# yukiteruono/pbsim3

Hardware: AMD Instinct MI355X
Metric: simulated bases/sec (higher is better)
Workload: dtype u8

## Files before the change

pbsim3_amd/csrc/deflate.hip:

```cpp
#include <hip/hip_runtime.h>
#include <stdint.h>
#include <stdlib.h>

#include "kernels.h"

namespace pbsim {

namespace {

constexpr int kChunk = DF_CHUNK;
constexpr int kThreads = 256;
constexpr int kSeg = kChunk / kThreads;
constexpr int kSegDw = kSeg / 4;
constexpr int kInDw = kChunk / 4 + kChunk / 128;
constexpr int kOutBytes = 33024;
constexpr int kOutDw = kOutBytes / 4;
constexpr int kSyms = 288;
constexpr uint32_t kPoly = 0xEDB88320u;
constexpr int kHeadBits = 18 * 8;
constexpr int kPrefixBits = 3 + 5 + 5 + 4 + 19 * 3;

constexpr int kClLenTab[19] = {3, 5, 4, 4, 4, 5, 5, 5, 5, 5, 5, 5, 4, 5, 5, 5, 5, 3, 3};
constexpr int kClOrderTab[19] = {16, 17, 18, 0, 8, 7, 9, 6, 10, 5, 11, 4, 12, 3, 13, 2, 14, 1, 15};
constexpr uint64_t pack_cl_len() {
  uint64_t v = 0;
  for (int s = 0; s < 19; ++s) v |= (uint64_t)kClLenTab[s] << (3 * s);
  return v;
}
constexpr uint64_t kClLenPacked = pack_cl_len();
__device__ __forceinline__ uint32_t cl_len(uint32_t s) { return (uint32_t)(kClLenPacked >> (3 * s)) & 7u; }
constexpr unsigned __int128 pack_prefix() {
  unsigned __int128 v = 1u | (2u << 1) | ((unsigned __int128)15 << 13);
  for (int i = 0; i < 19; ++i) v |= (unsigned __int128)kClLenTab[kClOrderTab[i]] << (17 + 3 * i);
  return v;
}
constexpr uint64_t kPrefixLo = (uint64_t)pack_prefix();
constexpr uint32_t kPrefixHi = (uint32_t)(pack_prefix() >> 64);

__device__ __forceinline__ uint32_t rev_bits(uint32_t code, uint32_t len) { return __brev(code) >> (32 - len); }

__device__ __forceinline__ uint32_t cl_code(uint32_t s) {
  uint32_t c, l = cl_len(s);
  if (l == 3) c = s == 0 ? 0 : s - 16;
  else if (l == 4) c = s == 12 ? 9 : 4 + s;
  else c = s == 1 ? 20 : s <= 11 ? 16 + s : 15 + s;
  return rev_bits(c, l);
}

__device__ __forceinline__ uint32_t gf2_mul(uint32_t a, uint32_t b) {
  uint32_t p = 0;
#pragma unroll
  for (int i = 0; i < 32; ++i) {
    p ^= b & (0u - ((a >> (31 - i)) & 1u));
    b = (b >> 1) ^ (kPoly & (0u - (b & 1u)));
  }
  return p;
}

struct BitWriter {
  uint32_t *out;
  uint32_t word, nb;
  uint64_t acc;
  __device__ __forceinline__ void init(uint32_t *o, uint32_t bitpos) {
    out = o;
    word = bitpos >> 5;
    nb = bitpos & 31;
    acc = 0;
  }
  __device__ __forceinline__ void put(uint32_t v, uint32_t k) {
    acc |= (uint64_t)v << nb;
    nb += k;
    if (nb >= 32) {
      atomicOr(&out[word++], (uint32_t)acc);
      acc >>= 32;
      nb -= 32;
    }
  }
  __device__ __forceinline__ void put64(uint64_t v, uint32_t k) {
    if (k > 32) {
      put((uint32_t)v, 32);
      put((uint32_t)(v >> 32), k - 32);
    } else {
      put((uint32_t)v, k);
    }
  }
  __device__ __forceinline__ void flush() {
    if (nb) atomicOr(&out[word], (uint32_t)acc);
  }
};

__device__ __forceinline__ void length_symbol(uint32_t L, uint32_t *sym, uint32_t *eb, uint32_t *ev) {
  const uint32_t v = L - 3;
  if (v < 8) {
    *sym = 257 + v;
    *eb = 0;
    *ev = 0;
  } else if (L == 258) {
    *sym = 285;
    *eb = 0;
    *ev = 0;
  } else {
    const uint32_t e = (31 - __clz(v)) - 2;
    *sym = 261 + 4 * e + ((v >> e) & 3);
    *eb = e;
    *ev = v & ((1u << e) - 1);
  }
}

__device__ __forceinline__ uint32_t block_scan_excl(uint32_t v, uint32_t *s_wave, uint32_t *total) {
  const int lane = threadIdx.x & 63, wave = threadIdx.x >> 6;
  uint32_t inc = v;
#pragma unroll
  for (int d = 1; d < 64; d <<= 1) {
    const uint32_t o = __shfl_up(inc, d, 64);
    if (lane >= d) inc += o;
  }
  __syncthreads();
  if (lane == 63) s_wave[wave] = inc;
  __syncthreads();
  uint32_t base = 0, tot = 0;
#pragma unroll
  for (int w = 0; w < kThreads / 64; ++w) {
    const uint32_t x = s_wave[w];
    if (w < wave) base += x;
    tot += x;
  }
  *total = tot;
  return base + inc - v;
}

struct Mask128 {
  uint64_t lo, hi;
};
__device__ __forceinline__ Mask128 m_and(Mask128 a, Mask128 b) { return {a.lo & b.lo, a.hi & b.hi}; }
__device__ __forceinline__ Mask128 m_or(Mask128 a, Mask128 b) { return {a.lo | b.lo, a.hi | b.hi}; }
__device__ __forceinline__ Mask128 m_not(Mask128 a) { return {~a.lo, ~a.hi}; }
template <int K>
__device__ __forceinline__ Mask128 m_shl(Mask128 a) { return {a.lo << K, (a.hi << K) | (a.lo >> (64 - K))}; }
template <int K>
__device__ __forceinline__ Mask128 m_shr(Mask128 a) { return {(a.lo >> K) | (a.hi << (64 - K)), a.hi >> K}; }
__device__ __forceinline__ uint32_t m_nibble(Mask128 a, int j) {
  return (uint32_t)((j < 16 ? a.lo >> (4 * j) : a.hi >> (4 * j - 64)) & 15u);
}
__device__ __forceinline__ int m_first(Mask128 a) { return a.lo ? __builtin_ctzll(a.lo) : 64 + __builtin_ctzll(a.hi); }
__device__ __forceinline__ Mask128 m_clear(Mask128 a, int pos) {
  if (pos < 64) a.lo &= ~(1ull << pos);
  else a.hi &= ~(1ull << (pos - 64));
  return a;
}
__device__ __forceinline__ int m_run(Mask128 m, int pos) {
  uint64_t lo, hi;
  if (pos == 0) {
    lo = m.lo;
    hi = m.hi;
  } else if (pos < 64) {
    lo = (m.lo >> pos) | (m.hi << (64 - pos));
    hi = m.hi >> pos;
  } else {
    lo = m.hi >> (pos - 64);
    hi = 0;
  }
  if (~lo) return __builtin_ctzll(~lo);
  return ~hi ? 64 + __builtin_ctzll(~hi) : 128;
}

struct SegTokens {
  Mask128 lit;
  Mask128 start;
  Mask128 cover;
};

__device__ __forceinline__ SegTokens seg_tokens(const uint32_t (&seg)[kSegDw], int seg_n, uint32_t prev_dword,
                                                bool chunk_start) {
  uint64_t e[2] = {0, 0};
  uint32_t pw = prev_dword;
#pragma unroll
  for (int j = 0; j < kSegDw; ++j) {
    const uint32_t w = seg[j];
    const uint32_t d = w ^ ((w << 8) | (pw >> 24));
    const uint32_t z = ~(((d & 0x7F7F7F7Fu) + 0x7F7F7F7Fu) | d | 0x7F7F7F7Fu);
    const uint32_t nib = (((z >> 7) * 0x00204081u) >> 21) & 15u;
    e[j >> 4] |= (uint64_t)nib << (4 * (j & 15));
    pw = w;
  }
  Mask128 valid;
  valid.lo = seg_n >= 64 ? ~0ull : (1ull << seg_n) - 1;
  valid.hi = seg_n >= 128 ? ~0ull : seg_n > 64 ? (1ull << (seg_n - 64)) - 1 : 0ull;
  Mask128 eq = {e[0] & valid.lo, e[1] & valid.hi};
  if (chunk_start) eq.lo &= ~1ull;
  const Mask128 r3 = m_and(eq, m_and(m_shr<1>(eq), m_shr<2>(eq)));
  SegTokens t;
  t.cover = m_or(r3, m_or(m_shl<1>(r3), m_shl<2>(r3)));
  t.start = m_and(t.cover, m_not(m_shl<1>(t.cover)));
  t.lit = m_and(valid, m_not(t.cover));
  return t;
}

constexpr int kSampleChunks = DF_SAMPLE_CHUNKS;
constexpr int kHdrDw = DF_TABLE_HDR_DW;

struct DfTable {
  uint32_t code[kSyms];
  uint32_t hdr_end_bits;
  uint32_t pad[3];
  uint32_t hdr[kHdrDw];
};
static_assert(sizeof(DfTable) <= DF_TABLE_BYTES, "DF_TABLE_BYTES too small");

__device__ __forceinline__ void load_chunk(const uint8_t *__restrict__ text, int64_t n_bytes, int64_t chunk, uint32_t *s_in,
                                           uint32_t (&seg)[kSegDw], int *n_out, int *seg_n_out, uint32_t *prev_dw) {
  const int tid = threadIdx.x;
  const int64_t base = chunk * (int64_t)kChunk;
  const int n = (int)((n_bytes - base) < (int64_t)kChunk ? (n_bytes - base) : (int64_t)kChunk);
  const uint4 *src4 = reinterpret_cast<const uint4 *>(text + base);
  for (int q = tid; q < kChunk / 16; q += kThreads) {
    uint4 v = make_uint4(0, 0, 0, 0);
    if (q * 16 < n) v = src4[q];
    const int d = q * 4;
    uint32_t *dst = &s_in[d + (d >> 5)];
    dst[0] = v.x;
    dst[1] = v.y;
    dst[2] = v.z;
    dst[3] = v.w;
  }
  __syncthreads();
  const int beg = tid * kSeg;
  *n_out = n;
  *seg_n_out = n - beg < 0 ? 0 : (n - beg < kSeg ? n - beg : kSeg);
#pragma unroll
  for (int j = 0; j < kSegDw; ++j) seg[j] = s_in[tid * (kSegDw + 1) + j];
  *prev_dw = tid ? s_in[tid * (kSegDw + 1) - 2] : 0u;
  __syncthreads();
}

__global__ __launch_bounds__(kThreads) void k_deflate_hist(const uint8_t *__restrict__ text, int64_t n_bytes,
                                                            uint32_t *__restrict__ hist) {
  __shared__ uint32_t s_in[kInDw];
  __shared__ uint32_t s_hist[3 * kSyms + 64];
  const int tid = threadIdx.x, lane = tid & 63;
  for (int i = tid; i < 3 * kSyms + 64; i += kThreads) s_hist[i] = 0;
  uint32_t seg[kSegDw], prev_dw;
  int n, seg_n;
  load_chunk(text, n_bytes, blockIdx.x, s_in, seg, &n, &seg_n, &prev_dw);
  const SegTokens tk = seg_tokens(seg, seg_n, prev_dw, tid == 0);
  const uint32_t copy = (uint32_t)(lane % 3) * kSyms, dummy = 3 * kSyms + lane;
#pragma unroll
  for (int j = 0; j < kSegDw; ++j) {
    const uint32_t nl = m_nibble(tk.lit, j);
    if (nl == 0) continue;
    const uint32_t w = seg[j];
#pragma unroll
    for (int k = 0; k < 4; ++k) atomicAdd(&s_hist[((nl >> k) & 1u) ? copy + ((w >> (8 * k)) & 255u) : dummy], 1u);
  }
  Mask128 st = tk.start;
  while (st.lo | st.hi) {
    const int pos = m_first(st);
    st = m_clear(st, pos);
    uint32_t sy, eb, ev;
    length_symbol((uint32_t)m_run(tk.cover, pos), &sy, &eb, &ev);
    atomicAdd(&s_hist[copy + sy], 1u);
  }
  __syncthreads();
  for (int i = tid; i < 286; i += kThreads) {
    const uint32_t f = s_hist[i] + s_hist[kSyms + i] + s_hist[2 * kSyms + i] + (i == 256 ? 1u : 0u);
    if (f) atomicAdd(&hist[i], f);
  }
}

__global__ __launch_bounds__(kThreads) void k_deflate_build(const uint32_t *__restrict__ hist, DfTable *__restrict__ tbl) {
  __shared__ uint32_t s_freq[kSyms], s_sfreq[kSyms], s_w[kSyms], s_code[kSyms];
  __shared__ uint16_t s_sorted[kSyms], s_par[kSyms], s_leafpar[kSyms], s_dep[kSyms];
  __shared__ uint8_t s_len[kSyms];
  __shared__ uint32_t s_cnt[16], s_first[16];
  __shared__ uint32_t s_img[4 + kHdrDw];
  const int tid = threadIdx.x;
  constexpr int m = 286;
  for (int i = tid; i < kSyms; i += kThreads) {
    s_freq[i] = i < m ? hist[i] + 1u : 0u;
    s_code[i] = 0;
    s_len[i] = 0;
  }
  for (int i = tid; i < 4 + kHdrDw; i += kThreads) s_img[i] = 0;
  if (tid < 16) s_cnt[tid] = 0;
  __syncthreads();
  for (int i = tid; i < m; i += kThreads) {
    const uint32_t fi = s_freq[i];
    uint32_t rank = 0;
    for (int u = 0; u < m; ++u) {
      const uint32_t g = s_freq[u];
      rank += (g < fi) | ((g == fi) & (u < i));
    }
    s_sorted[rank] = (uint16_t)i;
    s_sfreq[rank] = fi;
  }
  __syncthreads();
  if (tid == 0) {
    int leaf = 0, root = 0;
    for (int nxt = 0; nxt < m - 1; ++nxt) {
      uint32_t tot = 0;
      for (int k = 0; k < 2; ++k) {
        const bool take_leaf = leaf < m && (root >= nxt || s_sfreq[leaf] <= s_w[root]);
        if (take_leaf) {
          tot += s_sfreq[leaf];
          s_leafpar[leaf] = (uint16_t)nxt;
          ++leaf;
        } else {
          tot += s_w[root];
          s_par[root] = (uint16_t)nxt;
          ++root;
        }
      }
      s_w[nxt] = tot;
    }
    s_dep[m - 2] = 0;
    for (int i = m - 3; i >= 0; --i) s_dep[i] = s_dep[s_par[i]] + 1;
    for (int i = 0; i < m; ++i) {
      int d = s_dep[s_leafpar[i]] + 1;
      if (d > 15) d = 15;
      s_cnt[d] += 1;
    }
    uint32_t total = 0;
    for (int l = 1; l <= 15; ++l) total += s_cnt[l] << (15 - l);
    while (total > (1u << 15)) {
      s_cnt[15] -= 1;
      for (int l = 14; l >= 1; --l)
        if (s_cnt[l]) {
          s_cnt[l] -= 1;
          s_cnt[l + 1] += 2;
          break;
        }
      total -= 1;
    }
    int i = 0;
    for (int l = 15; l >= 1; --l)
      for (uint32_t k = 0; k < s_cnt[l]; ++k) s_len[s_sorted[i++]] = (uint8_t)l;
    uint32_t code = 0;
    s_cnt[0] = 0;
    for (int l = 1; l <= 15; ++l) {
      code = (code + s_cnt[l - 1]) << 1;
      s_first[l] = code;
    }
  }
  __syncthreads();
  for (int i = tid; i < m; i += kThreads) {
    const uint32_t l = s_len[i];
    uint32_t idx = 0;
    for (int u = 0; u < i; ++u) idx += s_len[u] == l;
    s_code[i] = rev_bits(s_first[l] + idx, l) | (l << 16);
  }
  __syncthreads();
  if (tid == 0) {
    BitWriter bw;
    bw.init(s_img, kHeadBits);
    bw.put64(kPrefixLo | ((uint64_t)(m - 257) << 3), 64);
    bw.put(kPrefixHi, kPrefixBits - 64);
    uint32_t bits = kHeadBits + kPrefixBits;
    int p = 0;
    const int npos = m + 1;
    while (p < npos) {
      const uint32_t v = p < m ? s_len[p] : 1u;
      bw.put(cl_code(v), cl_len(v));
      bits += cl_len(v);
      ++p;
      int r = 0;
      while (p + r < npos && (p + r < m ? s_len[p + r] : 1u) == v) ++r;
      while (r >= 3) {
        const int t = r < 6 ? r : 6;
        bw.put(cl_code(16) | ((uint32_t)(t - 3) << cl_len(16)), cl_len(16) + 2);
        bits += cl_len(16) + 2;
        r -= t;
        p += t;
      }
    }
    bw.flush();
    tbl->hdr_end_bits = bits;
  }
  __syncthreads();
  for (int i = tid; i < kSyms; i += kThreads) tbl->code[i] = s_code[i];
  for (int i = tid; i < kHdrDw; i += kThreads) tbl->hdr[i] = s_img[4 + i];
}

struct DfCtl {
  uint32_t ticket;
  uint32_t error;
  int64_t total;
};
static_assert(sizeof(DfCtl) == DF_CTL_BYTES, "DF_CTL_BYTES");

constexpr uint64_t kStSize = 1ull << 32, kStPrefix = 2ull << 32;
__device__ __forceinline__ uint64_t st_word(uint32_t epoch, uint64_t flag, uint32_t v) { return ((uint64_t)epoch << 34) | flag | v; }

__device__ __forceinline__ uint32_t look_back(const uint64_t *status, int64_t c, uint32_t epoch, int lane, uint32_t *error) {
  uint32_t sum = 0;
  int64_t hi = c - 1;
  for (uint32_t spins = 0;; spins++) {
    if (spins > (1u << 24)) {
      if (lane == 0) atomicOr(error, 1u);
      return sum;
    }
    const int64_t i = hi - lane;
    uint64_t w = 0;
    if (i >= 0) w = __hip_atomic_load(&status[i], __ATOMIC_RELAXED, __HIP_MEMORY_SCOPE_AGENT);
    const bool mine = i >= 0 && (uint32_t)(w >> 34) == epoch && ((w >> 32) & 3u) != 0;
    const uint64_t ready = __ballot(mine || i < 0);
    const uint64_t pref = __ballot(mine && ((w >> 32) & 3u) == 2u);
    const int k = ~ready ? __builtin_ctzll(~ready) : 64;
    const uint64_t usable = k >= 64 ? ~0ull : ((1ull << k) - 1);
    const uint64_t stop = pref & usable;
    if (stop) {
      const int e = __builtin_ctzll(stop);
      uint32_t v = (lane <= e && i >= 0) ? (uint32_t)w : 0u;
#pragma unroll
      for (int d = 32; d >= 1; d >>= 1) v += __shfl_xor(v, d, 64);
      return sum + v;
    }
    if (k == 0) {
      __builtin_amdgcn_s_sleep(2);
      continue;
    }
    uint32_t v = (lane < k && i >= 0) ? (uint32_t)w : 0u;
#pragma unroll
    for (int d = 32; d >= 1; d >>= 1) v += __shfl_xor(v, d, 64);
    sum += v;
    hi -= k;
    if (hi < 0) return sum;
  }
}

typedef uint32_t u32x4 __attribute__((ext_vector_type(4)));
__device__ __forceinline__ void store_member(uint8_t *dst, const uint32_t *s_img, uint32_t bytes, int tid) {
  const uint32_t head = min((uint32_t)((16u - ((uintptr_t)dst & 15u)) & 15u), bytes);
  const uint8_t *s8 = reinterpret_cast<const uint8_t *>(s_img);
  if ((uint32_t)tid < head) dst[tid] = s8[tid];
  const uint32_t nvec = (bytes - head) >> 4;
  const uint32_t sh = head & 3u, dw0 = head >> 2;
  u32x4 *d4 = reinterpret_cast<u32x4 *>(dst + head);
  for (uint32_t v = tid; v < nvec; v += kThreads) {
    const uint32_t *p = s_img + dw0 + 4u * v;
    const uint32_t a = p[0], b = p[1], c = p[2], d = p[3], e = p[4];
    u32x4 o;
    o.x = __builtin_amdgcn_alignbyte(b, a, sh);
    o.y = __builtin_amdgcn_alignbyte(c, b, sh);
    o.z = __builtin_amdgcn_alignbyte(d, c, sh);
    o.w = __builtin_amdgcn_alignbyte(e, d, sh);
    __builtin_nontemporal_store(o, &d4[v]);
  }
  const uint32_t done = head + 16u * nvec;
  if ((uint32_t)tid < bytes - done) dst[done + tid] = s8[done + tid];
}

__global__ __launch_bounds__(kThreads) void k_deflate_chunks(const uint8_t *__restrict__ text, int64_t n_bytes,
                                                              uint8_t *__restrict__ dense, uint64_t *__restrict__ status,
                                                              DfCtl *__restrict__ ctl, uint32_t epoch,
                                                              const uint32_t *__restrict__ crc_table,
                                                              const uint32_t *__restrict__ pow128, uint32_t x8rem,
                                                              const DfTable *__restrict__ tbl,
                                                              unsigned long long *__restrict__ prof) {
  __shared__ uint32_t s_in[kInDw];
  static_assert(kOutDw <= kInDw, "the output image must fit the input image");
  uint32_t *const s_out = s_in;
  __shared__ uint32_t s_code[kSyms];
  uint32_t *const s_crc = s_in;
  __shared__ uint32_t s_wave[kThreads / 64];
  __shared__ uint32_t s_misc[4];

  const int tid = threadIdx.x, lane = tid & 63;
  unsigned long long t_prev = prof ? wall_clock64() : 0;
  int phase = 0;
  auto mark = [&]() {
    if (prof && tid == 0) {
      const unsigned long long t = wall_clock64();
      atomicAdd(&prof[phase], t - t_prev);
      t_prev = t;
    }
    ++phase;
  };
  for (int i = tid; i < kSyms; i += kThreads) s_code[i] = i < 286 ? tbl->code[i] : 0u;
  if (tid < 4) s_misc[tid] = tid == 0 ? atomicAdd(&ctl->ticket, 1u) : 0u;
  __syncthreads();
  const int64_t chunk = s_misc[0];
  const int64_t n_chunks = (n_bytes + kChunk - 1) / kChunk;
  uint32_t seg[kSegDw], prev_dw;
  int n, seg_n;
  load_chunk(text, n_bytes, chunk, s_in, seg, &n, &seg_n, &prev_dw);
  const int beg = tid * kSeg;
  mark();
  for (int i = tid; i < kInDw; i += kThreads) s_in[i] = (i < 1024) ? crc_table[i] : 0u;
  __syncthreads();
  const SegTokens tk = seg_tokens(seg, seg_n, prev_dw, tid == 0);

  uint32_t tok_bits = 0;
  {
    uint32_t c = tid == 0 ? 0xFFFFFFFFu : 0u;
    const int full = seg_n >> 2;
#pragma unroll
    for (int j = 0; j < kSegDw; ++j) {
      if (j < full) {
        const uint32_t x = c ^ seg[j];
        c = s_crc[768 + (x & 255u)] ^ s_crc[512 + ((x >> 8) & 255u)] ^ s_crc[256 + ((x >> 16) & 255u)] ^ s_crc[x >> 24];
      } else if (j == full) {
        for (int k = 0; k < (seg_n & 3); ++k) c = s_crc[(c ^ (seg[j] >> (8 * k))) & 255u] ^ (c >> 8);
      }
    }
    const int q = n >> 7, r = n & 127;
    if (seg_n == kSeg && tid < q) {
      c = gf2_mul(c, pow128[q - tid - 1]);
      if (r) c = gf2_mul(c, x8rem);
    }
    if (seg_n == 0) c = 0;
#pragma unroll
    for (int d = 32; d >= 1; d >>= 1) c ^= __shfl_xor(c, d, 64);
    if (lane == 0) atomicXor(&s_misc[3], c);
  }
  mark();
  {
#pragma unroll
    for (int j = 0; j < kSegDw; ++j) {
      const uint32_t nl = m_nibble(tk.lit, j);
      if (nl == 0) continue;
      const uint32_t w = seg[j];
#pragma unroll
      for (int k = 0; k < 4; ++k)
        tok_bits += s_code[((nl >> k) & 1u) ? (w >> (8 * k)) & 255u : 287u] >> 16;
    }
    Mask128 st = tk.start;
    while (st.lo | st.hi) {
      const int pos = m_first(st);
      st = m_clear(st, pos);
      uint32_t sy, eb, ev;
      length_symbol((uint32_t)m_run(tk.cover, pos), &sy, &eb, &ev);
      tok_bits += (s_code[sy] >> 16) + eb + 1;
    }
  }
  uint32_t tok_total;
  const uint32_t tok_off = block_scan_excl(tok_bits, s_wave, &tok_total);
  const uint32_t hdr_end = tbl->hdr_end_bits;
  const uint32_t eob_len = s_code[256] >> 16;
  const uint32_t payload_bits = hdr_end - kHeadBits + tok_total + eob_len;
  const uint32_t payload_bytes = (payload_bits + 7) >> 3;
  const bool huff = (18 + payload_bytes + 8 <= (uint32_t)kOutBytes) && (payload_bytes < (uint32_t)n + 5);
  const uint32_t crc = s_misc[3] ^ 0xFFFFFFFFu;
  const uint32_t member = huff ? 18 + payload_bytes + 8 : 18 + 5 + (uint32_t)n + 8;
  if (tid == 0)
    __hip_atomic_store(&status[chunk], st_word(epoch, chunk == 0 ? kStPrefix : kStSize, member), __ATOMIC_RELAXED, __HIP_MEMORY_SCOPE_AGENT);
  mark();

  if (huff) {
    __syncthreads();
    for (int i = tid; i < 1024; i += kThreads) s_in[i] = 0;
    __syncthreads();
    if (tid < kHdrDw) s_out[4 + tid] = tbl->hdr[tid];
    if (tid == 0) {
      s_out[0] = 0x04088b1fu;
      s_out[1] = 0;
      s_out[2] = 0x0006ff00u;
      s_out[3] = 0x00024342u;
    }
    __syncthreads();
    if (tid == 0) atomicOr(&s_out[4], member - 1);
    mark();
    {
      BitWriter bw;
      bw.init(s_out, hdr_end + tok_off);
#pragma unroll
      for (int j = 0; j < kSegDw; ++j) {
        const uint32_t nl = m_nibble(tk.lit, j), ns = m_nibble(tk.start, j);
        if ((nl | ns) == 0) continue;
        const uint32_t w = seg[j];
        uint32_t c[4];
#pragma unroll
        for (int k = 0; k < 4; ++k) c[k] = s_code[((nl >> k) & 1u) ? (w >> (8 * k)) & 255u : 287u];
        uint32_t mv = 0, ml = 0, ks = 4;
        if (ns) {
          ks = (uint32_t)__builtin_ctz(ns);
          uint32_t sy, eb, ev;
          length_symbol((uint32_t)m_run(tk.cover, 4 * j + (int)ks), &sy, &eb, &ev);
          const uint32_t cm = s_code[sy];
          mv = (cm & 0xFFFFu) | (ev << (cm >> 16));
          ml = (cm >> 16) + eb + 1;
        }
        bw.put(ks == 0 ? mv : 0u, ks == 0 ? ml : 0u);
        {
          const uint32_t l0 = c[0] >> 16;
          bw.put((c[0] & 0xFFFFu) | ((c[1] & 0xFFFFu) << l0), l0 + (c[1] >> 16));
        }
        const bool mid = ks == 1 || ks == 2;
        bw.put(mid ? mv : 0u, mid ? ml : 0u);
        {
          const uint32_t l2 = c[2] >> 16;
          bw.put((c[2] & 0xFFFFu) | ((c[3] & 0xFFFFu) << l2), l2 + (c[3] >> 16));
        }
        bw.put(ks == 3 ? mv : 0u, ks == 3 ? ml : 0u);
      }
      bw.flush();
    }
    mark();
    if (tid == 0) {
      BitWriter bw;
      bw.init(s_out, hdr_end + tok_total);
      bw.put(s_code[256] & 0xFFFFu, eob_len);
      bw.flush();
      bw.init(s_out, (18 + payload_bytes) * 8);
      bw.put(crc, 32);
      bw.put((uint32_t)n, 32);
      bw.flush();
    }
    if (tid < 64 && chunk > 0) {
      const uint32_t excl = look_back(status, chunk, epoch, tid, &ctl->error);
      if (tid == 0) {
        s_misc[1] = excl;
        __hip_atomic_store(&status[chunk], st_word(epoch, kStPrefix, excl + member), __ATOMIC_RELAXED, __HIP_MEMORY_SCOPE_AGENT);
      }
    }
    __syncthreads();
    mark();
    const uint32_t off = s_misc[1];
    store_member(dense + off, s_out, member, tid);
    if (tid == 0 && chunk == n_chunks - 1) ctl->total = (int64_t)off + member;
    mark();
  } else {
    if (tid < 64 && chunk > 0) {
      const uint32_t excl = look_back(status, chunk, epoch, tid, &ctl->error);
      if (tid == 0) {
        s_misc[1] = excl;
        __hip_atomic_store(&status[chunk], st_word(epoch, kStPrefix, excl + member), __ATOMIC_RELAXED, __HIP_MEMORY_SCOPE_AGENT);
      }
    }
    __syncthreads();
    uint8_t *slot = dense + s_misc[1];
    if (tid == 0 && chunk == n_chunks - 1) ctl->total = (int64_t)s_misc[1] + member;
    if (tid == 0) {
      const uint8_t head[23] = {0x1f, 0x8b, 8,   4,   0,   0,
                                0,    0,    0,   0xff, 6,  0,
                                'B',  'C',  2,   0,   (uint8_t)((member - 1) & 255), (uint8_t)((member - 1) >> 8),
                                1,    (uint8_t)(n & 255), (uint8_t)(n >> 8), (uint8_t)(~n & 255), (uint8_t)((~n >> 8) & 255)};
      for (int i = 0; i < 23; ++i) slot[i] = head[i];
      uint8_t *t = slot + 23 + n;
      for (int i = 0; i < 4; ++i) t[i] = (uint8_t)(crc >> (8 * i));
      for (int i = 0; i < 4; ++i) t[4 + i] = (uint8_t)((uint32_t)n >> (8 * i));
    }
#pragma unroll
    for (int j = 0; j < kSegDw; ++j)
#pragma unroll
      for (int k = 0; k < 4; ++k)
        if (4 * j + k < seg_n) slot[23 + beg + 4 * j + k] = (uint8_t)(seg[j] >> (8 * k));
  }
}

uint32_t host_gf2_mul(uint32_t a, uint32_t b) {
  uint32_t p = 0;
  for (int i = 0; i < 32; ++i) {
    if (a & (0x80000000u >> i)) p ^= b;
    b = (b >> 1) ^ ((b & 1u) ? kPoly : 0u);
  }
  return p;
}

uint32_t host_xpow8(uint64_t nbytes) {
  uint32_t r = 0x80000000u, b = 0x00800000u;
  while (nbytes) {
    if (nbytes & 1) r = host_gf2_mul(r, b);
    b = host_gf2_mul(b, b);
    nbytes >>= 1;
  }
  return r;
}

}

void deflate_host_tables(uint32_t *crc_table, uint32_t *pow128) {
  for (uint32_t i = 0; i < 256; ++i) {
    uint32_t c = i;
    for (int k = 0; k < 8; ++k) c = (c >> 1) ^ ((c & 1u) ? kPoly : 0u);
    crc_table[i] = c;
  }
  for (int t = 1; t < 4; ++t)
    for (uint32_t i = 0; i < 256; ++i) {
      const uint32_t c = crc_table[(t - 1) * 256 + i];
      crc_table[t * 256 + i] = (c >> 8) ^ crc_table[c & 255u];
    }
  const uint32_t step = host_xpow8(128);
  uint32_t v = 0x80000000u;
  for (int k = 0; k < 256; ++k) {
    pow128[k] = v;
    v = host_gf2_mul(v, step);
  }
}

void launch_deflate_table(const uint8_t *text, int64_t n_bytes, uint32_t *hist, void *table, hipStream_t s) {
  if (n_bytes <= 0) return;
  const int64_t nch = (n_bytes + DF_CHUNK - 1) / DF_CHUNK;
  const int64_t ns = nch < kSampleChunks ? nch : kSampleChunks;
  const int64_t sample_bytes = ns * (int64_t)DF_CHUNK < n_bytes ? ns * (int64_t)DF_CHUNK : n_bytes;
  (void)hipMemsetAsync(hist, 0, 288 * sizeof(uint32_t), s);
  hipLaunchKernelGGL(k_deflate_hist, dim3((unsigned)ns), dim3(kThreads), 0, s, text, sample_bytes, hist);
  hipLaunchKernelGGL(k_deflate_build, dim3(1), dim3(kThreads), 0, s, (const uint32_t *)hist, reinterpret_cast<DfTable *>(table));
}

void launch_deflate(const uint8_t *text, int64_t n_bytes, uint64_t *status, void *ctl, uint32_t epoch, uint8_t *dense,
                    const uint32_t *d_crc_table, const uint32_t *d_pow128, const void *table, hipStream_t s,
                    unsigned long long *d_prof, hipEvent_t ev_begin, hipEvent_t ev_chunks_done) {
  if (n_bytes <= 0) return;
  const int64_t nch = (n_bytes + DF_CHUNK - 1) / DF_CHUNK;
  const uint32_t x8rem = host_xpow8((uint64_t)(n_bytes % DF_CHUNK) & 127u);
  (void)hipMemsetAsync(ctl, 0, DF_CTL_BYTES, s);
  if (ev_begin) (void)hipEventRecord(ev_begin, s);
  hipLaunchKernelGGL(k_deflate_chunks, dim3((unsigned)nch), dim3(kThreads), 0, s, text, n_bytes, dense, status,
                     reinterpret_cast<DfCtl *>(ctl), epoch & 0x3fffffffu, d_crc_table, d_pow128, x8rem,
                     reinterpret_cast<const DfTable *>(table), d_prof);
  if (ev_chunks_done) (void)hipEventRecord(ev_chunks_done, s);
}

}
```

pbsim3_amd/csrc/kernels.h:

```cpp
#pragma once
#include <hip/hip_runtime.h>
#include <stdint.h>

#include "modes.h"

namespace pbsim {

constexpr int kWG = 256;
constexpr int kLenBuckets = 4096;
constexpr int kBinPad = 16;
constexpr int kLenShift = 8;
constexpr int kScratchPad = 64;
constexpr int kMaxClasses = 64;
constexpr int32_t kWaveTransposed = 1 << 30;
constexpr int kHpTile = 4096;

enum : uint32_t {
  kErrScratchOverflow = 1u,
  kErrScratchBudget = 2u,
};

struct DeviceFlags {
  uint32_t error;
  uint32_t high_bytes;
  int64_t n_final;
  int64_t total_slots;
  int64_t scratch_need;
  int64_t sums[8];
  unsigned long long hpfreq[12];
  uint32_t need_q10;
  uint32_t max_rawlen;
};

struct RefView {
  const uint8_t *seq;
  const uint8_t *hp;
  int64_t len;
};


struct HeaderArgs {
  uint32_t seed, unit;
  int64_t first_read;
  int64_t n_reads;
  const int32_t *prob2len;
  int64_t len_rv;
  const uint8_t *prob2acc;
  int64_t acc_rv;
  int64_t ref_len;
  int64_t len_min;
  int64_t truncate_remaining;
  int32_t *rawlen, *len, *off;
  uint8_t *acc;
  uint32_t *max_rawlen;
  int32_t is_templ;
  const int32_t *read_unit;
  const int64_t *unit_len;
  const int32_t *unit_rank;
  const int32_t *off_table;
  const uint8_t *ssp;
  const int32_t *ssp_rv;
};

struct ChainState {
  int64_t remaining;
  int64_t total;
  int32_t made;
  int32_t done;
};

struct SortArgs {
  int64_t n_reads;
  int32_t pass_num;
  int32_t acc_lo, ncls;
  const int32_t *len;
  const uint8_t *acc;
  int32_t *hist;
  int32_t *bin_start;
  int32_t *bin_cursor;
  int32_t *class_start;
  int32_t coop_bucket;
  int32_t *coop_end;
  uint64_t coop_classes;
  int32_t *task_of_slot;
  int32_t *slot_of_task;
  int32_t *wave_cap;
  int64_t *wave_off;
  int64_t n_slots_max;
  int32_t *wg_hist, *wg_start;
  int32_t *wg_order;
  int32_t regions;
  int32_t cap_q8;
  int64_t scratch_bytes;
  DeviceFlags *flags;
};

struct WalkArgs {
  uint32_t seed, unit;
  int64_t first_read;
  int32_t pass_num;
  int32_t ncls;
  RefView ref;
  const int32_t *len, *off;
  const int64_t *read_base;
  const uint8_t *read_minus;
  const uint8_t *cls_blob;
  uint32_t stride, rows_off, init_off, tran_off, emis_off, freq_off, rv_off;
  const int32_t *class_start;
  const int32_t *task_of_slot;
  const int32_t *wg_order;
  int32_t mean_len;
  int32_t coop_min_len;
  int32_t coop_dynamic;
  int32_t cap_q8;
  const int32_t *coop_end;
  const int32_t *wave_cap;
  const int64_t *wave_off;
  uint8_t *scratch;
  int32_t *out_len, *maf_len, *nsub, *nins, *ndel;
  double *qsum;
  const uint32_t *sub_thre, *ins_thre, *del_thr;
  const double *qprob;
  DeviceFlags *flags;
};

struct SampleArgs {
  uint32_t seed, unit;
  int64_t first_read;
  int32_t n_lines;
  int32_t n_line_waves;
  int32_t n_coop_waves;
  int32_t n_coop_blocks;
  int64_t n_coop_slots;
  RefView ref;
  const uint8_t *quals;
  const int64_t *line_qoff;
  const int32_t *line_len;
  const int32_t *vbase;
  const int32_t *task_of_slot;
  const int32_t *wave_cap;
  const int64_t *wave_off;
  uint8_t *scratch;
  int32_t *span, *off;
  int32_t *out_len, *maf_len, *nsub, *nins, *ndel;
  double *qsum;
  const uint32_t *sub_thre, *ins_thre, *del_thr;
  const double *qprob;
  DeviceFlags *flags;
};

struct TextArgs {
  int64_t first_read;
  int64_t n_reads;
  int32_t pass_num;
  int32_t is_wgs;
  int32_t is_qs;
  uint32_t unit;
  int64_t ref_len;
  const int32_t *len, *off;
  const int32_t *out_len, *maf_len;
  const int32_t *slot_of_task;
  const int32_t *task_of_slot;
  int64_t *row_dst;
  const int32_t *wave_cap;
  const int64_t *wave_off;
  const uint8_t *scratch;
  const int64_t *read_text_off, *maf_text_off;
  int64_t *read_text_len, *maf_text_len;
  char *read_text, *maf_text;
  char id_prefix[64];
  int32_t id_prefix_len;
  char rq_text[32];
  int32_t rq_len;
  int32_t bam;
  uint32_t rq_bits;
  const int32_t *read_unit;
  const int64_t *unit_len;
  const char *unit_names;
  int32_t name_pad3;
  const uint8_t *read_minus;
  int32_t truth_bam;
  const int32_t *nsub, *nins, *ndel;
  int32_t *n_runs;
};

struct ReadArrays {
  uint8_t *seq, *qual;
  int32_t *ref_pos;
  int64_t *offsets;
  int64_t *read_number;
  int32_t *pass_index, *unit;
  uint8_t *strand;
  int64_t *ref_start;
  int32_t *ref_span, *n_sub, *n_ins, *n_del;
};

struct ExportArgs {
  int64_t first_read;
  int64_t n_reads;
  int64_t bases;
  int32_t pass_num;
  int32_t is_qs;
  uint32_t unit;
  const int32_t *len, *off;
  const int32_t *out_len, *maf_len, *nsub, *nins, *ndel;
  const int32_t *task_of_slot;
  const int32_t *wave_cap;
  const int64_t *wave_off;
  const uint8_t *scratch;
  const int32_t *read_unit;
  const uint8_t *read_minus;
  int64_t *task_off;
  ReadArrays out;
};

void launch_prepare_reference(uint8_t *seq, uint8_t *hp, int flag_hp11, int64_t len, int64_t *tile_first, int64_t *tile_last,
                              int64_t *carry_start, int64_t *carry_next, int keep_first_case, DeviceFlags *flags,
                              hipStream_t s);
void launch_squeeze_lines(const uint8_t *lines, int64_t bytes, uint8_t *dst, int64_t *tile_tmp, int64_t *scan_tmp, int64_t *total,
                          hipStream_t s);
void launch_header_wgs(const HeaderArgs &a, hipStream_t s);
void launch_header_trans(const HeaderArgs &a, hipStream_t s);
void launch_task_sort(const SortArgs &a, hipStream_t s);
void launch_chain_prepare(const HeaderArgs &a, int k, int32_t pass_num, const int32_t *task_of_slot, int32_t *masked,
                          int64_t n_slots_max, ChainState *chain, hipStream_t s);
void launch_chain_update(int k, int32_t pass_num, const int32_t *out_len, ChainState *chain, hipStream_t s);
void launch_chain_init(ChainState *chain, int64_t remaining, hipStream_t s);
void launch_walk_errhmm(const WalkArgs &a, int64_t n_slots_max, uint32_t lds_bytes, bool fast_rv, bool hp_bits,
                        hipStream_t s, int min_lds_kb);
constexpr int kCoopMaxStates = 31;
constexpr int kCoopWaves = 8;
void launch_walk_errhmm_coop(const WalkArgs &a, int n_wg, uint32_t lds_bytes, bool hp_bits, hipStream_t s);
int walk_errhmm_coop_resident(uint32_t lds_bytes, bool hp_bits);
constexpr int kQCoopMaxStates = 63;
void launch_walk_qshmm_coop(const WalkArgs &a, int n_wg, uint32_t lds_bytes, hipStream_t s);
void launch_qshmm_coop_qsum(const WalkArgs &a, int64_t n_slots_max, hipStream_t s);
void launch_walk_qshmm(const WalkArgs &a, int64_t n_slots_max, uint32_t lds_bytes, bool fast_rv, bool hp_bits,
                       hipStream_t s, int min_lds_kb);
void launch_walk_sample(const SampleArgs &a, bool hp_bits, hipStream_t s);
void launch_sample_qsum(const SampleArgs &a, hipStream_t s);
void launch_exclusive_scan_i64(const int64_t *in, int64_t *out, int64_t n, int64_t *tmp, int64_t *total, hipStream_t s);
void launch_gather_pass0_scan(const int32_t *out_len, int64_t n_reads, int32_t pass_num, int64_t *cum, int64_t *tmp,
                              int64_t *total, hipStream_t s);
void launch_quota_cut(const int64_t *cum, const int32_t *rawlen, int64_t n_reads, int64_t len_total_before,
                      int64_t quota, int force_all, DeviceFlags *flags, hipStream_t s);
void launch_cigar_count(const TextArgs &a, int64_t n_slots_max, const DeviceFlags *flags, hipStream_t s);
void launch_text_sizes(const TextArgs &a, DeviceFlags *flags, hipStream_t s);
void launch_text_emit(const TextArgs &a, int64_t n_slots_max, const DeviceFlags *flags, hipStream_t s);
void launch_export_sizes(const ExportArgs &a, DeviceFlags *flags, int64_t *scan_tmp, hipStream_t s);
void launch_export(const ExportArgs &a, int64_t n_slots_max, const DeviceFlags *flags, hipStream_t s);

#define DF_CHUNK 32768
#define DF_SLOT (DF_CHUNK + 64)
#define DF_PIECE_CHUNKS 8192
#define DF_SAMPLE_CHUNKS 64
#define DF_TABLE_HDR_DW 96
#define DF_TABLE_BYTES 2048
void deflate_host_tables(uint32_t *crc_table , uint32_t *pow128 );
void launch_deflate_table(const uint8_t *text, int64_t n_bytes, uint32_t *hist, void *table, hipStream_t s);
#define DF_CTL_BYTES 16
void launch_deflate(const uint8_t *text, int64_t n_bytes, uint64_t *status, void *ctl, uint32_t epoch, uint8_t *dense,
                    const uint32_t *d_crc_table, const uint32_t *d_pow128, const void *table, hipStream_t s,
                    unsigned long long *d_prof = nullptr ,
                    hipEvent_t ev_begin = nullptr, hipEvent_t ev_chunks_done = nullptr );

struct InflateMember {
  int64_t in_off, out_off;
  int32_t in_len, out_len;
  uint32_t crc, pad;
};
enum InflateStatus : int32_t {
  kInfOk = 0,
  kInfBlockType,
  kInfStoredLen,
  kInfTooMany,
  kInfClSet,
  kInfRepeat,
  kInfNoEob,
  kInfLitSet,
  kInfDistSet,
  kInfLitCode,
  kInfDistCode,
  kInfTooFar,
  kInfTruncated,
  kInfTrailing,
  kInfCrc,
  kInfLength,
  kInfCount
};
const char *inflate_reason(int32_t status);
void launch_inflate(const uint8_t *in, const InflateMember *members, int64_t n_members, uint8_t *out, int32_t *status,
                    const uint32_t *d_crc_table, const uint32_t *d_pow128, hipStream_t s);

constexpr int kSpTile = 1024;
inline int64_t sp_tiles(int64_t b0, int64_t b1) { return b1 > b0 ? (b1 - (b0 & ~(int64_t)(kSpTile - 1)) + kSpTile - 1) / kSpTile : 0; }
void launch_sp_count(const uint8_t *buf, int64_t b0, int64_t b1, int64_t *tile_count, int32_t *nul, hipStream_t s);
void launch_sp_lines(const uint8_t *buf, int64_t b0, int64_t b1, int phase, const int64_t *tile_base, uint32_t *rec_start,
                     uint32_t *rec_end, hipStream_t s);
void launch_sp_sums(const uint8_t *buf, const uint32_t *rec_start, const uint32_t *rec_end, int64_t n_rec, int32_t len_min,
                    int32_t len_max, double acc_min, double acc_max, const double *qprob , int32_t *rec_len,
                    double *accuracy, int64_t *padded, hipStream_t s);
void launch_sp_pool(const uint8_t *buf, const uint32_t *rec_start, const int32_t *rec_len, const int64_t *padded, const int64_t *off,
                    int64_t n_rec, uint8_t *pool, hipStream_t s);

enum : int32_t { kSbCounted = 0, kSbSkipped = 1, kSbNoQual = 2 };
void launch_sb_sums(const uint8_t *buf, const uint64_t *rec, int64_t n_rec, int32_t len_min, int32_t len_max, double acc_min, double acc_max,
                    const double *qprob , uint32_t *qual_at, int32_t *rec_len, int32_t *status, double *accuracy,
                    int64_t *padded, hipStream_t s);
void launch_sb_pool(const uint8_t *buf, const uint64_t *rec, const uint32_t *qual_at, const int32_t *rec_len, const int64_t *padded,
                    const int64_t *off, int64_t n_rec, uint8_t *pool, hipStream_t s);

}
```

Measured before the change: 58.47 billion.

## Add register-resident fast Huffman lookup for common literal bytes via byte permute

The table builder now picks, for each of 8 slots keyed on the low 3 bits of a byte, the most frequent literal whose code fits in 8 bits. It stores check bytes, code lengths and codes in the table. The deflate kernel uses v_perm and sad_u8 to look up whole dwords of literals in registers, and falls back to the shared-memory s_code lookup only when some lane misses. The goal is to cut LDS lookups in both the bit-count pass and the emit pass, which suits low-entropy DNA text. It also shrinks the zeroing of the output buffer to the member size and adds asm barriers to steer register allocation. The trade-offs are extra ALU work per dword and wave-divergent fallback paths.

```diff
diff --git a/pbsim3_amd/csrc/deflate.hip b/pbsim3_amd/csrc/deflate.hip
--- a/pbsim3_amd/csrc/deflate.hip
+++ b/pbsim3_amd/csrc/deflate.hip
@@ -142,6 +142,11 @@
 __device__ __forceinline__ uint32_t m_nibble(Mask128 a, int j) {
   return (uint32_t)((j < 16 ? a.lo >> (4 * j) : a.hi >> (4 * j - 64)) & 15u);
 }
+constexpr uint32_t kNibbleSpread = 0x00204081u;
+__device__ __forceinline__ uint32_t lit_bytes(uint32_t nib, uint32_t spread = kNibbleSpread) {
+  const uint32_t b = __umul24(nib, spread) & 0x01010101u;
+  return (b << 8) - b;
+}
 __device__ __forceinline__ int m_first(Mask128 a) { return a.lo ? __builtin_ctzll(a.lo) : 64 + __builtin_ctzll(a.hi); }
 __device__ __forceinline__ Mask128 m_clear(Mask128 a, int pos) {
   if (pos < 64) a.lo &= ~(1ull << pos);
@@ -204,6 +209,9 @@
   uint32_t hdr_end_bits;
   uint32_t pad[3];
   uint32_t hdr[kHdrDw];
+  uint32_t fast_chk[DF_TABLE_FAST_SLOTS / 4];
+  uint32_t fast_len[DF_TABLE_FAST_SLOTS / 4];
+  uint32_t fast_code[DF_TABLE_FAST_SLOTS / 4];
 };
 static_assert(sizeof(DfTable) <= DF_TABLE_BYTES, "DF_TABLE_BYTES too small");
 
@@ -378,6 +386,21 @@
   __syncthreads();
   for (int i = tid; i < kSyms; i += kThreads) tbl->code[i] = s_code[i];
   for (int i = tid; i < kHdrDw; i += kThreads) tbl->hdr[i] = s_img[4 + i];
+  if (tid < 2) {
+    uint32_t chk = 0, len = 0, code = 0;
+    for (int k = 0; k < 4; ++k) {
+      const int v = 4 * tid + k;
+      int best = -1;
+      for (int b = v; b < 256; b += 8)
+        if (s_len[b] <= 8 && (best < 0 || s_freq[b] > s_freq[best])) best = b;
+      chk |= (uint32_t)(best < 0 ? (v ^ 1) : best) << (8 * k);
+      len |= (best < 0 ? 0u : (uint32_t)s_len[best]) << (8 * k);
+      code |= (best < 0 ? 0u : s_code[best] & 0xFFu) << (8 * k);
+    }
+    tbl->fast_chk[tid] = chk;
+    tbl->fast_len[tid] = len;
+    tbl->fast_code[tid] = code;
+  }
 }
 
 struct DfCtl {
@@ -485,9 +508,12 @@
   load_chunk(text, n_bytes, chunk, s_in, seg, &n, &seg_n, &prev_dw);
   const int beg = tid * kSeg;
   mark();
-  for (int i = tid; i < kInDw; i += kThreads) s_in[i] = (i < 1024) ? crc_table[i] : 0u;
+  for (int i = tid; i < 1024; i += kThreads) s_in[i] = crc_table[i];
   __syncthreads();
   const SegTokens tk = seg_tokens(seg, seg_n, prev_dw, tid == 0);
+  const uint32_t chk_lo = tbl->fast_chk[0], chk_hi = tbl->fast_chk[1];
+  const uint32_t len_lo = tbl->fast_len[0], len_hi = tbl->fast_len[1];
+  const uint32_t code_lo = tbl->fast_code[0], code_hi = tbl->fast_code[1];
 
   uint32_t tok_bits = 0;
   {
@@ -513,15 +539,24 @@
     if (lane == 0) atomicXor(&s_misc[3], c);
   }
   mark();
+  uint32_t fast = 0;
   {
 #pragma unroll
     for (int j = 0; j < kSegDw; ++j) {
       const uint32_t nl = m_nibble(tk.lit, j);
-      if (nl == 0) continue;
       const uint32_t w = seg[j];
-#pragma unroll
-      for (int k = 0; k < 4; ++k)
-        tok_bits += s_code[((nl >> k) & 1u) ? (w >> (8 * k)) & 255u : 287u] >> 16;
+      const uint32_t sel = w & 0x07070707u;
+      const uint32_t lm = lit_bytes(nl);
+      const bool f = ((__builtin_amdgcn_perm(chk_hi, chk_lo, sel) ^ w) & lm) == 0u;
+      fast |= (f ? 1u : 0u) << j;
+      if (f) tok_bits = __builtin_amdgcn_sad_u8(__builtin_amdgcn_perm(len_hi, len_lo, sel) & lm, 0u, tok_bits);
+      const bool slow = !f;
+      if (!__any(slow)) continue;
+      if (slow) {
+#pragma unroll
+        for (int k = 0; k < 4; ++k)
+          tok_bits += s_code[((nl >> k) & 1u) ? (w >> (8 * k)) & 255u : 287u] >> 16;
+      }
     }
     Mask128 st = tk.start;
     while (st.lo | st.hi) {
@@ -532,6 +567,7 @@
       tok_bits += (s_code[sy] >> 16) + eb + 1;
     }
   }
+  asm volatile("" : "+v"(fast));
   uint32_t tok_total;
   const uint32_t tok_off = block_scan_excl(tok_bits, s_wave, &tok_total);
   const uint32_t hdr_end = tbl->hdr_end_bits;
@@ -547,7 +583,8 @@
 
   if (huff) {
     __syncthreads();
-    for (int i = tid; i < 1024; i += kThreads) s_in[i] = 0;
+    const int n_zero = min((int)(member >> 2) + 3, kInDw);
+    for (int i = tid; i < n_zero; i += kThreads) s_out[i] = 0;
     __syncthreads();
     if (tid < kHdrDw) s_out[4 + tid] = tbl->hdr[tid];
     if (tid == 0) {
@@ -562,14 +599,27 @@
     {
       BitWriter bw;
       bw.init(s_out, hdr_end + tok_off);
+      uint32_t m7 = 0x07070707u, k81 = kNibbleSpread, e_len_lo = len_lo, e_len_hi = len_hi;
+      asm volatile("" : "+s"(m7), "+s"(k81), "+s"(e_len_lo), "+s"(e_len_hi));
 #pragma unroll
       for (int j = 0; j < kSegDw; ++j) {
         const uint32_t nl = m_nibble(tk.lit, j), ns = m_nibble(tk.start, j);
         if ((nl | ns) == 0) continue;
         const uint32_t w = seg[j];
+        const bool f = (fast >> j) & 1u;
         uint32_t c[4];
-#pragma unroll
-        for (int k = 0; k < 4; ++k) c[k] = s_code[((nl >> k) & 1u) ? (w >> (8 * k)) & 255u : 287u];
+        {
+          const uint32_t sel = w & m7, lm = lit_bytes(nl, k81);
+          const uint32_t cd = __builtin_amdgcn_perm(code_hi, code_lo, sel) & lm, ln = __builtin_amdgcn_perm(e_len_hi, e_len_lo, sel) & lm;
+#pragma unroll
+          for (int k = 0; k < 4; ++k) c[k] = ((cd >> (8 * k)) & 255u) | (((ln >> (8 * k)) & 255u) << 16);
+        }
+        if (__any(!f)) {
+          if (!f) {
+#pragma unroll
+            for (int k = 0; k < 4; ++k) c[k] = s_code[((nl >> k) & 1u) ? (w >> (8 * k)) & 255u : 287u];
+          }
+        }
         uint32_t mv = 0, ml = 0, ks = 4;
         if (ns) {
           ks = (uint32_t)__builtin_ctz(ns);
@@ -639,11 +689,13 @@
       for (int i = 0; i < 4; ++i) t[i] = (uint8_t)(crc >> (8 * i));
       for (int i = 0; i < 4; ++i) t[4 + i] = (uint8_t)((uint32_t)n >> (8 * i));
     }
+    int left = seg_n;
+    asm volatile("" : "+v"(left));
 #pragma unroll
     for (int j = 0; j < kSegDw; ++j)
 #pragma unroll
       for (int k = 0; k < 4; ++k)
-        if (4 * j + k < seg_n) slot[23 + beg + 4 * j + k] = (uint8_t)(seg[j] >> (8 * k));
+        if (4 * j + k < left) slot[23 + beg + 4 * j + k] = (uint8_t)(seg[j] >> (8 * k));
   }
 }
 
diff --git a/pbsim3_amd/csrc/kernels.h b/pbsim3_amd/csrc/kernels.h
--- a/pbsim3_amd/csrc/kernels.h
+++ b/pbsim3_amd/csrc/kernels.h
@@ -255,6 +255,7 @@
 #define DF_PIECE_CHUNKS 8192
 #define DF_SAMPLE_CHUNKS 64
 #define DF_TABLE_HDR_DW 96
+#define DF_TABLE_FAST_SLOTS 8
 #define DF_TABLE_BYTES 2048
 void deflate_host_tables(uint32_t *crc_table , uint32_t *pow128 );
 void launch_deflate_table(const uint8_t *text, int64_t n_bytes, uint32_t *hist, void *table, hipStream_t s);
```

After: 58.25 billion. About the same (-0.4%).
